# miguelmartin75/txt2vid

Measured on AMD Instinct MI355X. Metric: TGANv2 GAN train throughput (G+D steps x global batch), 16x64x64 videos/sec, higher is better.
Workload: dtype f32; 1 GPU; BASELINE configs[1]: unconditional TGANv2 16x64x64x1, per-GPU batch 32, fp32, RSGAN + GP 0.5, Adam 2e-4 (0.5,0.999), 1 D + 1 G step, subsample_input pyramid 8/16/32/64; global_batch=32, per_gpu_batch=32, parallelism=dp1

## Files before the change

include/t2v_hip.h:

```cpp
#ifndef T2V_HIP_H
#define T2V_HIP_H

#include <stdint.h>

#ifdef __cplusplus
extern "C" {
#endif

#define T2V_OK 0
#define T2V_EINVAL (-1)
#define T2V_ELAUNCH (-2)

#define T2V_MAX_TAPS 27

typedef struct {
    int32_t N, Cin, D, H, W, Cout;
    int32_t ntaps;
    int8_t dz[T2V_MAX_TAPS], dy[T2V_MAX_TAPS], dx[T2V_MAX_TAPS];
    int8_t pad_[3];
} t2v_conv_geom;

#define T2V_MAX_GROUPS 8
typedef struct {
    const float* x;
// ... 56 lines not shown
    int8_t pad_[5];
    int64_t tap_stride;
    int64_t split_stride;
} t2v_wgrad_src;
typedef struct {
    float* dw;
    float* dbias;
    int64_t CoCi;
    int32_t T, Cout, nsrc;
    int32_t accum, accum_bias;
    int32_t kind;
    int32_t block_begin, nblocks;
    int32_t tap_major;
    int32_t pad_;
    t2v_wgrad_src src[T2V_WGRAD_MAX_SRC];
} t2v_wgrad_dest;
int t2v_conv_wgrad_grouped_partial(const t2v_conv_group* groups, int ngroups, int Cin, int Cout, int kD, int kH, int kW,
                                   float* slab, int want_bias, int flags, t2v_wgrad_src* out_src, void* stream);
int t2v_wgrad_dest_bytes(void);
int t2v_wgrad_reduce_multi(const void* table , int ndest, int total_blocks, void* stream);

int t2v_conv_fwd_plan(const t2v_conv_group* groups, int ngroups, int Cin, int Cout, int flags, int32_t* out);
int t2v_conv_wgrad_plan(const t2v_conv_group* groups, int ngroups, int Cin, int Cout, int kD, int kH, int kW, int32_t* out);
int64_t t2v_conv_wgrad_grouped_bias_slab_floats(const t2v_conv_group* groups, int ngroups, int Cin, int Cout, int kD,
                                                int kH, int kW);
int t2v_conv_wgrad_grouped_bias(const t2v_conv_group* groups, int ngroups, int Cin, int Cout, int kD, int kH, int kW,
                                float* dw, float* dbias, float* slab, int flags, void* stream);

int t2v_pack_weight_bf16(const float* w, void* wpb, int Cout, int Cin, int T, const int32_t* taps, int ntaps, int mode, void* stream);
int t2v_conv_fwd_grouped_bf16_ok(const t2v_conv_group* groups, int ngroups, int Cin, int Cout);
int t2v_conv_fwd_bf16_plan(const t2v_conv_group* groups, int ngroups, int Cin, int Cout, int flags, int32_t* out);
int t2v_conv_fwd_grouped_bf16(const t2v_conv_group* groups, int ngroups, int Cin, int Cout, const void* wpb, const float* bias,
                              float* ws, int flags, void* stream);

int64_t t2v_channel_sum_ws_floats(int N, int C, int64_t S);
int t2v_channel_sum(const float* x, float* out, float* ws, int N, int C, int64_t S, int accum, void* stream);
int64_t t2v_channel_sum_grouped_ws_floats(const t2v_conv_group* groups, int ngroups, int C);
int t2v_channel_sum_grouped(const t2v_conv_group* groups, int ngroups, int C, float* out, float* ws, int accum, void* stream);

int t2v_relu(const float* x, float* y, int64_t n, void* stream);
int t2v_relu_mask(const float* g, const float* x, float* gx, int64_t n, void* stream);
int t2v_add(const float* a, const float* b, float* y, int64_t n, void* stream);
int t2v_axpby(float alpha, const float* a, float beta, const float* b, float* y, int64_t n, void* stream);
int t2v_scale_dev(const float* s, float mul, const float* a, float* y, int64_t n, void* stream);
int t2v_dot(const float* a, const float* b, float* out, float* ws , int64_t n, int accum, void* stream);
int t2v_fill(float* y, float v, int64_t n, void* stream);
// ... 225 lines not shown
```

txt2vid_amd/_lib.py:

```python
import ctypes as C
import os

_HERE = os.path.dirname(os.path.abspath(__file__))
LIB_PATH = os.environ.get('T2V_LIB') or os.path.join(_HERE, 'csrc', 'libt2v_hip.so')

MAX_TAPS = 27


class ConvGeom(C.Structure):
    _fields_ = [('N', C.c_int32), ('Cin', C.c_int32), ('D', C.c_int32), ('H', C.c_int32), ('W', C.c_int32),
                ('Cout', C.c_int32), ('ntaps', C.c_int32),
                ('dz', C.c_int8 * MAX_TAPS), ('dy', C.c_int8 * MAX_TAPS), ('dx', C.c_int8 * MAX_TAPS),
                ('pad_', C.c_int8 * 3)]


class ConvGroup(C.Structure):
    _fields_ = [('x', C.c_void_p), ('y', C.c_void_p), ('mask', C.c_void_p), ('N', C.c_int32), ('D', C.c_int32), ('H', C.c_int32), ('W', C.c_int32),
                ('ntaps', C.c_int32), ('dstride', C.c_int32), ('ydstride', C.c_int32), ('yoff', C.c_int32), ('Dy', C.c_int32),
                ('dz', C.c_int8 * MAX_TAPS), ('dy', C.c_int8 * MAX_TAPS), ('dx', C.c_int8 * MAX_TAPS), ('widx', C.c_int8 * MAX_TAPS)]


class AdamJob(C.Structure):
    _fields_ = [('p', C.c_void_p), ('g', C.c_void_p), ('m', C.c_void_p), ('v', C.c_void_p), ('n', C.c_int64)]

# ... 52 lines not shown
_F = C.c_float
_I3 = C.POINTER(C.c_int32)
_G = C.POINTER(ConvGeom)

SIGNATURES = {
    't2v_pack_weight': [_P, _P, _I, _I, _I, _I3, _I, _I, _P],
    't2v_pack_job_bytes': [],
    't2v_pack_multi': [_P, _I, _I, _P],
    't2v_pack_weight_into': [_P, _P, _I, _I, _I, _I3, _I, _I, _I, _I, _I, _I, _P],
    't2v_conv_fwd': [_P, _P, _P, _P, _P, _G, _I, _P],
    't2v_conv_fwd_ws_floats': [_G],
    't2v_conv_wgrad_slab_floats': [_G, _I],
    't2v_conv_fwd_grouped_ws_floats': [_P, _I, _I, _I],
    't2v_conv_fwd_grouped': [_P, _I, _I, _I, _P, _P, _P, _I, _P],
    't2v_conv_wgrad_grouped_slab_floats': [_P, _I, _I, _I, _I, _I, _I],
    't2v_conv_fwd_plan': [_P, _I, _I, _I, _I, _I3],
    't2v_nonlocal_ok': [_I, _I],
    't2v_nonlocal_fwd': [_P, _P, _P, _P, _P, _I, _I, _I, _I, _I, _P],
    't2v_nonlocal_bwd': [_P, _P, _P, _P, _P, _P, _P, _P, _P, _P, _I, _I, _I, _I, _I, _P],
    't2v_conv_wgrad_grouped_partial': [_P, _I, _I, _I, _I, _I, _I, _P, _I, _I, _P, _P],
    't2v_wgrad_dest_bytes': [],
    't2v_wgrad_reduce_multi': [_P, _I, _I, _P],
    't2v_conv_wgrad_plan': [_P, _I, _I, _I, _I, _I, _I, _I3],
    't2v_pack_weight_bf16': [_P, _P, _I, _I, _I, _P, _I, _I, _P],
    't2v_conv_fwd_grouped_bf16_ok': [_P, _I, _I, _I],
    't2v_conv_fwd_bf16_plan': [_P, _I, _I, _I, _I, _I3],
    't2v_conv_fwd_grouped_bf16': [_P, _I, _I, _I, _P, _P, _P, _I, _P],
    't2v_conv_wgrad_grouped': [_P, _I, _I, _I, _I, _I, _I, _P, _P, _I, _P],
    't2v_conv_wgrad_grouped_bias_slab_floats': [_P, _I, _I, _I, _I, _I, _I],
    't2v_conv_wgrad_grouped_bias': [_P, _I, _I, _I, _I, _I, _I, _P, _P, _P, _I, _P],
    't2v_conv_wgrad': [_P, _P, _P, _P, _G, _I3, _I, _I, _P],
    't2v_channel_sum_ws_floats': [_I, _I, _L],
    't2v_channel_sum': [_P, _P, _P, _I, _I, _L, _I, _P],
    't2v_channel_sum_grouped_ws_floats': [_P, _I, _I],
    't2v_channel_sum_grouped': [_P, _I, _I, _P, _P, _I, _P],
    't2v_relu': [_P, _P, _L, _P],
    't2v_relu_mask': [_P, _P, _P, _L, _P],
    't2v_add': [_P, _P, _P, _L, _P],
    't2v_axpby': [_F, _P, _F, _P, _P, _L, _P],
    't2v_scale_dev': [_P, _F, _P, _P, _L, _P],
    't2v_dot': [_P, _P, _P, _P, _L, _I, _P],
    't2v_fill': [_P, _F, _L, _P],
    't2v_tanh': [_P, _P, _L, _P],
    't2v_tanh_bwd': [_P, _P, _P, _L, _P],
    't2v_avgpool3d': [_P, _P, _P, _I, _I, _I, _I, _I, _I, _I, _I3, _I3, _I3, _P],
    't2v_avgpool3d_bwd': [_P, _P, _I, _I, _I, _I, _I, _I, _I, _I3, _I3, _I3, _P],
# ... 125 lines not shown
```

txt2vid_amd/csrc/conv.hip:

```cpp
#include <hip/hip_runtime.h>
#include <stdint.h>
#include "../../include/t2v_hip.h"

typedef float f32x16 __attribute__((ext_vector_type(16)));

#ifdef T2V_STAMPS
__device__ unsigned long long* g_stamps = nullptr;
__device__ unsigned int g_stamps_cap = 0;
extern "C" int t2v_stamps_set(void* buf, unsigned int cap_records) {
    if (hipMemcpyToSymbol(HIP_SYMBOL(g_stamps), &buf, sizeof(buf)) != hipSuccess) return -1;
    if (hipMemcpyToSymbol(HIP_SYMBOL(g_stamps_cap), &cap_records, sizeof(cap_records)) != hipSuccess) return -1;
    return 0;
}
__device__ __forceinline__ unsigned long long stamp_now() {
    unsigned long long t;
    __builtin_amdgcn_sched_barrier(0);
    asm volatile("s_memtime %0\n\ts_waitcnt lgkmcnt(0)" : "=s"(t) :: "memory");
    __builtin_amdgcn_sched_barrier(0);
    return t;
}
#define STAMP(v) const unsigned long long v = stamp_now()
#define STAMP_ACC(acc, a, b) acc += (b) - (a)
#else
#define STAMP(v)
// ... 3503 lines not shown
            const int slot = col / Cin, ci = col - slot * Cin;
            float* ps = slab + ((size_t)split * live.n + slot) * Cout * Cin + ci;
#pragma unroll
            for (int r = 0; r < 16; ++r) {
                const int co = co0 + wco * 32 + (r & 3) + 8 * (r >> 2) + 4 * hi;
                if (co < Cout) ps[(size_t)co * Cin] = acc[r];
            }
        } else if (col == 31 && bias_slab != nullptr) {
#pragma unroll
            for (int r = 0; r < 16; ++r) {
                const int co = co0 + wco * 32 + (r & 3) + 8 * (r >> 2) + 4 * hi;
                if (co < Cout) bias_slab[(size_t)split * Cout + co] = acc[r];
            }
        }
    }
}

#define W3_AP (WG_BK + 1)
#define W3_BP (WG_BK + 3)
struct LiveRows { int8_t r[9]; int32_t n; };

#define W3_XP (WG_BK + 3)

template <bool BF16>
__global__ __launch_bounds__(256, BF16 ? 4 : 0) void conv_wgrad3_kernel(const WGroupTable tab, float* __restrict__ slab, const int Cin,
                                                          const int Cout, const int kD, const int kH, const int flags,
                                                          const int chunks_per_split, const LiveRows live,
                                                          float* __restrict__ bias_slab) {
    constexpr int LDS_A = BF16 ? 64 * B16_KP * 2 : 64 * W3_AP * 4;
    constexpr int LDS_B = BF16 ? 3 * 64 * B16_KP * 2 : 3 * 64 * W3_XP * 4;
    __shared__ __attribute__((aligned(16))) unsigned char lds_raw[LDS_A + LDS_B];
    float* const As = reinterpret_cast<float*>(lds_raw);
    float* const Bs = reinterpret_cast<float*>(lds_raw + LDS_A);
    __bf16* const Ah = reinterpret_cast<__bf16*>(lds_raw);
    __bf16* const Bh = reinterpret_cast<__bf16*>(lds_raw + LDS_A);
    const int tid = threadIdx.x, lane = tid & 63, wave = tid >> 6;
    const int l31 = lane & 31, hi = lane >> 5;
    const int wco = wave & 1, wci = wave >> 1;
    const int nco_t = (Cout + 63) / 64;
    const int co0 = (blockIdx.x % nco_t) * 64, ci0 = (blockIdx.x / nco_t) * 64;
    const int lin = xcd_remap((int)(blockIdx.y + blockIdx.z * gridDim.y), (int)(gridDim.y * gridDim.z));
    const int rslot = lin % (int)gridDim.y;
    const int split = lin / (int)gridDim.y;
    const int krow = live.r[rslot];
    const int dz = krow / kH - kD / 2, dy = krow % kH - kH / 2;
    const float relu_floor = (flags & T2V_CONV_RELU_IN) ? 0.f : -__builtin_inff();
    const int ml = tid & 31, rl = tid >> 5;
    const bool full = co0 + 64 <= Cout && ci0 + 64 <= Cin;

    f32x16 acc0, acc1, acc2;
#pragma unroll
    for (int r = 0; r < 16; ++r) { acc0[r] = 0.f; acc1[r] = 0.f; acc2[r] = 0.f; }

// ... 78 lines not shown
                ra[p] = __builtin_bit_cast(float, __builtin_amdgcn_raw_buffer_load_b32(g_y, oa, p * sty, 0));
                rb[p] = __builtin_bit_cast(float, __builtin_amdgcn_raw_buffer_load_b32(g_x, ob, p * st, 0));
            }
        } else {
#pragma unroll
            for (int p = 0; p < 8; ++p) {
                const int co = co0 + rl + p * 8, ci = ci0 + rl + p * 8;
                ra[p] = __builtin_bit_cast(float, __builtin_amdgcn_raw_buffer_load_b32(
                    g_y, (gbase + (uint32_t)(co < Cout ? co : Cout - 1) * uDHWo) * 4u, 0, 0));
                rb[p] = __builtin_bit_cast(float, __builtin_amdgcn_raw_buffer_load_b32(
                    g_x, (xb + (uint32_t)(ci < Cin ? ci : Cin - 1) * uDHW) * 4u, 0, 0));
            }
        }
        const uint32_t xb_l = __shfl(xb, 0, 64), xb_r = __shfl(xb, 31, 64);
        if (tid < 128) {
            const int row = tid >> 1, side = tid & 1;
            const int ci = ci0 + row;
            const uint32_t base = side ? (((pm2 >> 31) & 1u) ? xb_r + 1u : 0u) : ((pm0 & 1u) ? xb_l - 1u : 0u);
            rh = __builtin_bit_cast(float, __builtin_amdgcn_raw_buffer_load_b32(
                g_x, (base + (uint32_t)(ci < Cin ? ci : Cin - 1) * uDHW) * 4u, 0, 0));
        }
    };

    if (q0 < q1) load_chunk(q0);
    for (int q = q0; q < q1; ++q) {
        {
            const bool v0 = (((uint64_t)pm0 >> (ml + 1)) & 1u) != 0;
            const bool v1 = ((pm1 >> ml) & 1u) != 0;
            const bool v2 = ((((uint64_t)pm2 << 1) >> ml) & 1u) != 0;
            if (do_bias) {
#pragma unroll
                for (int p = 0; p < 8; ++p) bsum[p] += pend_mv ? ra[p] : 0.f;
            }
            if constexpr (BF16) {
                const int c_m1 = ml + 1, c_p1 = ml >= 1 ? ml - 1 : 33;
#pragma unroll
                for (int p = 0; p < 8; ++p) {
                    const int row = rl + p * 8;
                    float a = ra[p], v = fmaxf(rb[p], relu_floor);
                    if (!full) {
                        a = (co0 + row < Cout) ? a : 0.f;
                        v = (ci0 + row < Cin) ? v : 0.f;
                    }
                    Ah[row * B16_KP + ml] = (__bf16)a;
                    Bh[(0 * 64 + row) * B16_KP + c_m1] = (__bf16)(v0 ? v : 0.f);
                    Bh[(1 * 64 + row) * B16_KP + ml] = (__bf16)(v1 ? v : 0.f);
// ... 49 lines not shown
#pragma unroll
        for (int k2 = 0; k2 < WG_BK / 2; ++k2) {
            const float a = qa[k2 * 2];
            const float b0 = qb[0 * 64 * W3_XP + k2 * 2];
            const float b1 = qb[1 * 64 * W3_XP + k2 * 2];
            const float b2 = qb[2 * 64 * W3_XP + k2 * 2];
            acc0 = __builtin_amdgcn_mfma_f32_32x32x2f32(a, b0, acc0, 0, 0, 0);
            acc1 = __builtin_amdgcn_mfma_f32_32x32x2f32(a, b1, acc1, 0, 0, 0);
            acc2 = __builtin_amdgcn_mfma_f32_32x32x2f32(a, b2, acc2, 0, 0, 0);
        }
        }
        __syncthreads();
    }
    if (do_bias) {
#pragma unroll
        for (int p = 0; p < 8; ++p) {
            float v = bsum[p];
#pragma unroll
            for (int o = 16; o > 0; o >>= 1) v += __shfl_xor(v, o, 64);
            const int co = co0 + rl + p * 8;
            if (ml == 0 && co < Cout) bias_slab[(size_t)split * Cout + co] = v;
        }
    }
    const int ci = ci0 + wci * 32 + l31;
    if (ci < Cin) {
        const size_t CoCi = (size_t)Cout * Cin;
        float* ps = slab + ((size_t)split * (live.n * 3) + (size_t)rslot * 3) * CoCi + ci;
#pragma unroll
        for (int r = 0; r < 16; ++r) {
            const int co = co0 + wco * 32 + (r & 3) + 8 * (r >> 2) + 4 * hi;
            if (co < Cout) {
                ps[(size_t)co * Cin] = acc0[r];
                ps[CoCi + (size_t)co * Cin] = acc1[r];
                ps[2 * CoCi + (size_t)co * Cin] = acc2[r];
            }
        }
    }
}


__global__ __launch_bounds__(256, 4) void conv_pool_wgrad_kernel(const WGroupTable tab, float* __restrict__ slab, const int Cin,
                                                              const int Cout, const int chunks_per_split, const LiveRows live,
                                                              float* __restrict__ bias_slab) {
    constexpr int PA = WG_BK + 1;
    __shared__ __attribute__((aligned(16))) float As[64 * PA];
    __shared__ __attribute__((aligned(16))) float Bs[3 * 64 * PA];
    const int tid = threadIdx.x, lane = tid & 63, wave = tid >> 6;
    const int l31 = lane & 31, hi = lane >> 5;
    const int wco = wave & 1, wci = wave >> 1;
    const int nco_t = (Cout + 63) / 64;
    const int co0 = (blockIdx.x % nco_t) * 64, ci0 = (blockIdx.x / nco_t) * 64;
    const int lin = xcd_remap((int)(blockIdx.y + blockIdx.z * gridDim.y), (int)(gridDim.y * gridDim.z));
    const int rslot = lin % (int)gridDim.y;
    const int split = lin / (int)gridDim.y;
    const int krow = live.r[rslot];
    const int dz = krow / 3 - 1, dy = krow % 3 - 1;
    const int ml = tid & 31, rl = tid >> 5;
    const bool full = co0 + 64 <= Cout && ci0 + 64 <= Cin;

    f32x16 acc0, acc1, acc2;
#pragma unroll
    for (int r = 0; r < 16; ++r) { acc0[r] = 0.f; acc1[r] = 0.f; acc2[r] = 0.f; }

    const int nchunks = tab.chunk_start[tab.n];
    const int q0 = split * chunks_per_split;
    int q1 = q0 + chunks_per_split;
    if (q1 > nchunks) q1 = nchunks;

    float ra[8], rb1[8];
// ... 62 lines not shown
        const uint32_t uVp = (uint32_t)gVp, uVn = (uint32_t)gVn;
        if (full) {
            const uint32_t oa = (gbase + (uint32_t)(co0 + rl) * uVn) * 4u, ob = (xb + (uint32_t)(ci0 + rl) * uVp) * 4u;
            const int st = 32 * gVp, sty = 32 * gVn;
#pragma unroll
            for (int p = 0; p < 8; ++p) {
                ra[p] = __builtin_bit_cast(float, __builtin_amdgcn_raw_buffer_load_b32(g_y, oa, p * sty, 0));
                rb2[p] = __builtin_bit_cast(float2, __builtin_amdgcn_raw_buffer_load_b64(g_x, ob, p * st, 0));
                rb1[p] = __builtin_bit_cast(float, __builtin_amdgcn_raw_buffer_load_b32(g_x, ob + 8u, p * st, 0));
            }
        } else {
#pragma unroll
            for (int p = 0; p < 8; ++p) {
                const int co = co0 + rl + p * 8, ci = ci0 + rl + p * 8;
                ra[p] = __builtin_bit_cast(float, __builtin_amdgcn_raw_buffer_load_b32(
                    g_y, (gbase + (uint32_t)(co < Cout ? co : Cout - 1) * uVn) * 4u, 0, 0));
                const uint32_t ob = (xb + (uint32_t)(ci < Cin ? ci : Cin - 1) * uVp) * 4u;
                rb2[p] = __builtin_bit_cast(float2, __builtin_amdgcn_raw_buffer_load_b64(g_x, ob, 0, 0));
                rb1[p] = __builtin_bit_cast(float, __builtin_amdgcn_raw_buffer_load_b32(g_x, ob + 8u, 0, 0));
            }
        }
    };

    if (q0 < q1) load_chunk(q0);
    for (int q = q0; q < q1; ++q) {
        {
            if (do_bias) {
#pragma unroll
                for (int p = 0; p < 8; ++p) bsum[p] += pend_mv ? ra[p] : 0.f;
            }
            float* pa = &As[rl * PA + ml];
            float* pb = &Bs[rl * PA + ml];
#pragma unroll
            for (int p = 0; p < 8; ++p) {
                float a = pend_mv ? ra[p] : 0.f;
                float v0 = pend_vc ? rb2[p].x : 0.f, v1 = pend_vc ? rb2[p].y : 0.f, v2 = pend_vc ? rb1[p] : 0.f;
                if (!full) {
                    const int row = rl + p * 8;
                    a = (co0 + row < Cout) ? a : 0.f;
                    const bool ok = ci0 + row < Cin;
                    v0 = ok ? v0 : 0.f; v1 = ok ? v1 : 0.f; v2 = ok ? v2 : 0.f;
                }
                pa[p * 8 * PA] = a;
                pb[(0 * 64 + p * 8) * PA] = v0;
                pb[(1 * 64 + p * 8) * PA] = v1;
                pb[(2 * 64 + p * 8) * PA] = v2;
// ... 4 lines not shown
        const float* qa = &As[(wco * 32 + l31) * PA + hi];
        const float* qb = &Bs[(wci * 32 + l31) * PA + hi];
#pragma unroll
        for (int k2 = 0; k2 < WG_BK / 2; ++k2) {
            const float a = qa[k2 * 2];
            const float b0 = qb[0 * 64 * PA + k2 * 2];
            const float b1 = qb[1 * 64 * PA + k2 * 2];
            const float b2 = qb[2 * 64 * PA + k2 * 2];
            acc0 = __builtin_amdgcn_mfma_f32_32x32x2f32(a, b0, acc0, 0, 0, 0);
            acc1 = __builtin_amdgcn_mfma_f32_32x32x2f32(a, b1, acc1, 0, 0, 0);
            acc2 = __builtin_amdgcn_mfma_f32_32x32x2f32(a, b2, acc2, 0, 0, 0);
        }
        __syncthreads();
    }
    if (do_bias) {
#pragma unroll
        for (int p = 0; p < 8; ++p) {
            float v = bsum[p];
#pragma unroll
            for (int o = 16; o > 0; o >>= 1) v += __shfl_xor(v, o, 64);
            const int co = co0 + rl + p * 8;
            if (ml == 0 && co < Cout) bias_slab[(size_t)split * Cout + co] = v;
        }
    }
    const int ci = ci0 + wci * 32 + l31;
    if (ci < Cin) {
        const size_t CoCi = (size_t)Cout * Cin;
        float* ps = slab + ((size_t)split * (live.n * 3) + (size_t)rslot * 3) * CoCi + ci;
#pragma unroll
        for (int r = 0; r < 16; ++r) {
            const int co = co0 + wco * 32 + (r & 3) + 8 * (r >> 2) + 4 * hi;
            if (co < Cout) {
                ps[(size_t)co * Cin] = acc0[r];
                ps[CoCi + (size_t)co * Cin] = acc1[r];
                ps[2 * CoCi + (size_t)co * Cin] = acc2[r];
            }
        }
    }
}


__device__ __forceinline__ void bias_slab_reduce(const float* __restrict__ bias_slab, float* __restrict__ dbias, int S, int Cout,
                                                 int accum) {
    for (int co = threadIdx.x; co < Cout; co += 256) {
        float v0 = 0.f, v1 = 0.f, v2 = 0.f, v3 = 0.f;
        int s = 0;
// ... 167 lines not shown
    for (int i = 0; i < 2; ++i)
#pragma unroll
        for (int j = 0; j < 2; ++j) {
            const int ci = ci0 + wci * 64 + j * 32 + l31;
#pragma unroll
            for (int r = 0; r < 16; ++r) {
                const int co = co0 + wco * 64 + i * 32 + (r & 3) + 8 * (r >> 2) + 4 * hi;
                if (co < Cout && ci < Cin) out[(size_t)co * Cin + ci] = acc[i][j][r];
            }
        }
    if (do_bias) {
        float* red = As;
        *reinterpret_cast<float4*>(&red[r8 * WGM_AP + c4]) = bsum;
        __syncthreads();
        if (tid < 128 && co0 + tid < Cout) {
            float v = 0.f;
#pragma unroll
            for (int k = 0; k < 8; ++k) v += red[k * WGM_AP + tid];
            bias_slab[(size_t)split * Cout + co0 + tid] = v;
        }
    }
}

struct WgradPlan { int S, cps; uint32_t live; int nlive; long nchunks; bool rows3; uint32_t liverows; int nrows; bool strided; bool gemm; bool thin; };

static bool build_wtable(const t2v_conv_group* groups, int ngroups, int Cin, int Cout, int kD, int kH, int kW, bool need_ptrs,
                         WGroupTable& tab, WgradPlan& p) {
    if (!groups || ngroups < 1 || ngroups > T2V_MAX_GROUPS || Cin < 1 || Cout < 1) return false;
    if ((kD != 1 && kD != 3) || (kH != 1 && kH != 3) || (kW != 1 && kW != 3)) return false;
    long nch = 0, maxMC = 0;
    bool strided = false;
    p.live = 0;
    tab.n = ngroups;
    for (int i = 0; i < ngroups; ++i) {
        const t2v_conv_group& g = groups[i];
        if (need_ptrs && (!g.x || !g.y)) return false;
        if (g.N < 1 || g.D < 1 || g.H < 1 || g.W < 1 || g.dstride < 0 || g.dstride > 2 || g.ydstride > 1 || g.ydstride < 0) return false;
        if (g.dstride == 2) strided = true;
        const long M = (long)g.N * g.D * g.H * g.W;
        if (M * (long)(Cin > Cout ? Cin : Cout) >= (1L << 30)) return false;
        if (M * (long)(Cin > Cout ? Cin : Cout) > maxMC) maxMC = M * (long)(Cin > Cout ? Cin : Cout);
        tab.g[i] = g;
        tab.chunk_start[i] = (int32_t)nch;
        nch += ((long)g.N * out_frames(g) * g.H * g.W + WG_BK - 1) / WG_BK;
        for (int a = 0; a < kD; ++a) for (int b = 0; b < kH; ++b) for (int c = 0; c < kW; ++c) {
            const int dz = a - kD / 2, dy = b - kH / 2, dx = c - kW / 2;
// ... 69 lines not shown
}

static void fill_wgrad_plan(int Cin, int Cout, const WgradPlan& p, int32_t* out) {
    const long tiles = (long)((Cout + 63) / 64) * ((Cin + 63) / 64);
    out[0] = p.gemm ? 3 : p.rows3 ? 2 : p.thin ? 4 : (Cin < 64 ? 1 : 0);
    out[1] = p.S;
    out[2] = p.cps;
    out[3] = p.nlive;
    out[4] = ((long)Cout * Cin <= 16384 && p.S >= 16) ? 1 : 0;
    if (p.gemm) { out[5] = (int32_t)((long)((Cout + 127) / 128) * ((Cin + 127) / 128) * p.S); return; }
    if (p.thin) { out[5] = (int32_t)((long)((Cout + 63) / 64) * p.S); return; }
    out[5] = (int32_t)((p.rows3 ? tiles * p.nrows : Cin < 64 ? (long)((Cout + 63) / 64) * (((long)p.nlive * Cin + 63) / 64)
                                                              : tiles * p.nlive) * p.S);
}
extern "C" int t2v_conv_wgrad_plan(const t2v_conv_group* groups, int ngroups, int Cin, int Cout, int kD, int kH, int kW,
                                   int32_t* out) {
    WGroupTable tab;
    WgradPlan p;
    if (!out || !build_wtable(groups, ngroups, Cin, Cout, kD, kH, kW, false, tab, p)) return T2V_EINVAL;
    fill_wgrad_plan(Cin, Cout, p, out);
    return T2V_OK;
}

extern "C" int64_t t2v_channel_sum_grouped_ws_floats(const t2v_conv_group* groups, int ngroups, int C);
extern "C" int t2v_channel_sum_grouped(const t2v_conv_group* groups, int ngroups, int C, float* out, float* ws, int accum, void* stream);

static int64_t wgrad_bias_extra(const t2v_conv_group* groups, int ngroups, int Cin, int Cout, const WgradPlan& p) {
    return (int64_t)p.S * Cout;
}
extern "C" int64_t t2v_conv_wgrad_grouped_bias_slab_floats(const t2v_conv_group* groups, int ngroups, int Cin, int Cout, int kD,
                                                           int kH, int kW) {
    WGroupTable tab;
    WgradPlan p;
    if (!build_wtable(groups, ngroups, Cin, Cout, kD, kH, kW, false, tab, p)) return T2V_EINVAL;
    return (int64_t)p.S * p.nlive * Cout * Cin + wgrad_bias_extra(groups, ngroups, Cin, Cout, p);
}

static int wgrad_impl(const t2v_conv_group* groups, int ngroups, int Cin, int Cout, int kD, int kH, int kW, float* dw,
                      float* dbias, float* slab, int flags, void* stream, t2v_wgrad_src* out_src = nullptr);
extern "C" int t2v_conv_wgrad_grouped(const t2v_conv_group* groups, int ngroups, int Cin, int Cout, int kD, int kH, int kW,
                                      float* dw, float* slab, int flags, void* stream) {
    return wgrad_impl(groups, ngroups, Cin, Cout, kD, kH, kW, dw, nullptr, slab, flags, stream);
}
extern "C" int t2v_conv_wgrad_grouped_bias(const t2v_conv_group* groups, int ngroups, int Cin, int Cout, int kD, int kH, int kW,
                                           float* dw, float* dbias, float* slab, int flags, void* stream) {
    if (!dbias) return T2V_EINVAL;
// ... 36 lines not shown
    for (int i = 0; i < ngroups; ++i) {
        int live_g = 0;
        for (int a = 0; a < kD; ++a) for (int b = 0; b < kH; ++b) for (int c = 0; c < kW; ++c) {
            const int dz = a - kD / 2, dy = b - kH / 2, dx = c - kW / 2;
            if (!((groups[i].D == 1 && dz) || (groups[i].H == 1 && dy) || (groups[i].W == 1 && dx))) ++live_g;
        }
        flops += 2.0 * (double)groups[i].N * out_frames(groups[i]) * groups[i].H * groups[i].W * Cout * Cin * live_g;
    }
    {
        ProfScope prof(1, flops, s, p.nchunks * WG_BK, Cin, Cout, live.n, ngroups, p.S);
        int32_t plan_[8] = {-1, -1, -1, -1, -1, -1, -1, -1};
        fill_wgrad_plan(Cin, Cout, p, plan_);
        plan_[6] = ((flags & T2V_CONV_BF16) && !p.gemm && (p.rows3 || Cin >= 64)) ? 1 : 0;
        plan_[7] = p.strided ? 1 : 0;
        ProfScope::set_plan(plan_, 8);
        if (p.gemm) {
            dim3 grid((unsigned)(((Cout + 127) / 128) * ((Cin + 127) / 128)), 1u, (unsigned)p.S);
            T2V_LAUNCH_PROF(conv_wgrad_gemm_kernel, grid, dim3(256), 0, s, tab, slab, Cin, Cout, flags, p.cps,
                            dbias ? bias_part : (float*)nullptr);
        } else if (p.rows3) {
            dim3 grid((unsigned)(((Cout + 63) / 64) * ((Cin + 63) / 64)), (unsigned)lrows.n, (unsigned)p.S);
            if (flags & T2V_CONV_BF16)
                T2V_LAUNCH_PROF(conv_wgrad3_kernel<true>, grid, dim3(256), 0, s, tab, slab, Cin, Cout, kD, kH, flags, p.cps, lrows,
                                dbias ? bias_part : (float*)nullptr);
            else
                T2V_LAUNCH_PROF(conv_wgrad3_kernel<false>, grid, dim3(256), 0, s, tab, slab, Cin, Cout, kD, kH, flags, p.cps, lrows,
                                dbias ? bias_part : (float*)nullptr);
        } else if (Cin < 64 && p.thin) {
            dim3 grid((unsigned)((Cout + 63) / 64), 1u, (unsigned)p.S);
            T2V_LAUNCH_PROF(conv_wgrad_thin_kernel, grid, dim3(256), 0, s, tab, slab, Cin, Cout, T, kH, kW, flags, p.cps, live,
                            dbias ? bias_part : (float*)nullptr);
        } else if (Cin < 64) {
            dim3 grid((unsigned)(((Cout + 63) / 64) * ((live.n * Cin + 63) / 64)), 1u, (unsigned)p.S);
            T2V_LAUNCH_PROF(conv_wgrad_cols_kernel, grid, dim3(256), 0, s, tab, slab, Cin, Cout, T, kH, kW, flags, p.cps, live,
                            dbias ? bias_part : (float*)nullptr);
        } else {
            dim3 grid((unsigned)(((Cout + 63) / 64) * ((Cin + 63) / 64)), (unsigned)live.n, (unsigned)p.S);
            if (flags & T2V_CONV_BF16)
                T2V_LAUNCH_PROF(conv_wgrad_bf16_kernel, grid, dim3(256), 0, s, tab, slab, Cin, Cout, T, kH, kW, flags, p.cps, live,
                                dbias ? bias_part : (float*)nullptr);
            else
                T2V_LAUNCH_PROF(conv_wgrad_kernel, grid, dim3(256), 0, s, tab, slab, Cin, Cout, T, kH, kW, flags, p.cps, live,
                                dbias ? bias_part : (float*)nullptr);
        }
    }
    int st = launch_status();
// ... 242 lines not shown
    if ((!dw && !out_src) || !slab || !build_pool_wtable(groups, ngroups, Cin, Cout, kD, true, tab, p)) return T2V_EINVAL;
    hipStream_t s = (hipStream_t)stream;
    float* bias_part = slab + (size_t)p.S * p.nlive * Cout * Cin;
    const int T = kD * 9;
    TapMap map;
    for (int t = 0; t < T2V_MAX_TAPS; ++t) map.j[t] = -1;
    LiveRows lrows;
    lrows.n = 0;
    for (int r = 0; r < 9; ++r) lrows.r[r] = 0;
    for (int r = 0; r < 9; ++r)
        if ((p.liverows >> r) & 1u) {
            const int rw = kD == 3 ? r : r - 3;
            for (int c = 0; c < 3; ++c) map.j[rw * 3 + c] = lrows.n * 3 + c;
            lrows.r[lrows.n++] = (int8_t)r;
        }
    double flops = 0;
    for (int i = 0; i < ngroups; ++i) flops += 2.0 * (double)pool_rows(groups[i]) * Cout * Cin * (groups[i].dstride ? 27 : 9);
    {
        ProfScope prof(1, flops, s, p.nchunks * WG_BK, Cin, Cout, p.nlive, ngroups, p.S);
        int32_t plan_[8] = {11, p.S, p.cps, p.nlive, ((long)Cout * Cin <= 16384 && p.S >= 16) ? 1 : 0,
                            (int32_t)((long)((Cout + 63) / 64) * ((Cin + 63) / 64) * p.nrows * p.S), 0, 0};
        ProfScope::set_plan(plan_, 8);
        dim3 grid((unsigned)(((Cout + 63) / 64) * ((Cin + 63) / 64)), (unsigned)lrows.n, (unsigned)p.S);
        T2V_LAUNCH_PROF(conv_pool_wgrad_kernel, grid, dim3(256), 0, s, tab, slab, Cin, Cout, p.cps, lrows, want_bias ? bias_part : (float*)nullptr);
    }
    int st = launch_status();
    if (st) return st;
    if (out_src) {
        out_src->slab = slab;
        out_src->bias_slab = want_bias ? bias_part : (const float*)nullptr;
        out_src->ntaps = p.nlive;
        out_src->S = p.S;
        out_src->tap_stride = (int64_t)Cout * Cin;
        out_src->split_stride = (int64_t)p.nlive * Cout * Cin;
        for (int t = 0; t < T2V_MAX_TAPS; ++t) out_src->map[t] = (int8_t)(t < T ? map.j[t] : -1);
        return T2V_OK;
    }
    const float* bias_in = want_bias ? bias_part : (const float*)nullptr;
    const int accum_bias = (flags & T2V_CONV_ACCUM_BIAS) ? 1 : 0;
    const long CoCi = (long)Cout * Cin;
    ProfScope prof2(2, 0.0, s, CoCi, Cin, Cout, T, p.nlive, p.S);
    if (CoCi <= 16384 && p.S >= 16)
        T2V_LAUNCH_PROF(wgrad_reduce_small_kernel, dim3((unsigned)((CoCi + 63) / 64), (unsigned)T), dim3(256), 0, s, slab, dw, CoCi, T,
                   p.nlive, p.S, map, (flags & T2V_CONV_ACCUM) ? 1 : 0, bias_in, dbias, Cout, accum_bias);
    else
        T2V_LAUNCH_PROF(wgrad_reduce_kernel, dim3((unsigned)((CoCi + 63) / 64)), dim3(256), 0, s, slab, dw, CoCi, T, p.nlive, p.S, map,
                   (flags & T2V_CONV_ACCUM) ? 1 : 0, bias_in, dbias, Cout, accum_bias);
// ... 7 lines not shown
extern "C" int t2v_pool_conv_wgrad_partial(const t2v_conv_group* groups, int ngroups, int Cin, int Cout, int kD, float* slab,
                                           int want_bias, int flags, t2v_wgrad_src* out_src, void* stream) {
    if (!out_src) return T2V_EINVAL;
    return pool_wgrad_impl(groups, ngroups, Cin, Cout, kD, nullptr, nullptr, want_bias != 0, slab, flags, stream, out_src);
}
extern "C" int t2v_pool_conv_plan(int what, const t2v_conv_group* groups, int ngroups, int Cin, int Cout, int32_t* out) {
    if (!out) return T2V_EINVAL;
    for (int i = 0; i < 8; ++i) out[i] = 0;
    if (what == 0 || what == 1) {
        GroupTable tab;
        PoolPlan p;
        if (!(what == 0 ? build_pool_fwd(groups, ngroups, Cin, Cout, false, tab, p) : build_pool_dgrad(groups, ngroups, Cin, Cout, false, tab, p)))
            return T2V_EINVAL;
        const bool db = what == 0 ? pool_fwd_db() : pool_dgrad_db();
        out[0] = what == 0 ? 9 : 10; out[1] = 64; out[2] = 64; out[3] = db ? 16 : 32; out[4] = 1; out[5] = p.vecb ? 1 : 0; out[6] = db ? 2 : 1; out[7] = p.S;
        return T2V_OK;
    }
    if (what == 2) {
        WGroupTable tab;
        WgradPlan p;
        if (!build_pool_wtable(groups, ngroups, Cin, Cout, 3, false, tab, p)) return T2V_EINVAL;
        out[0] = 11; out[1] = p.S; out[2] = p.cps; out[3] = p.nlive; out[4] = ((long)Cout * Cin <= 16384 && p.S >= 16) ? 1 : 0;
        out[5] = (int32_t)((long)((Cout + 63) / 64) * ((Cin + 63) / 64) * p.nrows * p.S);
        return T2V_OK;
    }
    return T2V_EINVAL;
}

extern "C" int t2v_wgrad_dest_bytes(void) { return (int)sizeof(t2v_wgrad_dest); }


__global__ __launch_bounds__(256) void wgrad_reduce_multi_kernel(const t2v_wgrad_dest* __restrict__ table, int ndest) {
    __shared__ __attribute__((aligned(16))) float tile[256 * T2V_MAX_TAPS];
    __shared__ __attribute__((aligned(16))) float part[4][256];
    __shared__ int s_dest;
    if (threadIdx.x == 0) {
        int lo = 0, hi = ndest - 1;
        while (lo < hi) {
            const int mid = (lo + hi + 1) >> 1;
            if (table[mid].block_begin <= (int)blockIdx.x) lo = mid; else hi = mid - 1;
        }
        s_dest = lo;
    }
    __syncthreads();
    const t2v_wgrad_dest& d = table[s_dest];
    const int b = (int)blockIdx.x - d.block_begin;
// ... 304 lines not shown
```

Before: 3004 videos/s.

## Double-buffer fp32 wgrad and pool-wgrad kernels with half-chunk software pipelining

Adds a double-buffered variant of the fp32 3-row wgrad kernel and the pooled wgrad kernel. Each K chunk is split into two half-chunk rounds with two LDS buffers, so global loads for the next round are issued between MFMAs and staged into the other buffer. This needs only one barrier per round, where the single-buffer version waits on a load then stage then compute sequence. It is on by default through T2V_WGRAD_DB and adds launch bounds of 4, which may raise register pressure. A plan query reporting the chosen form is also exposed.

After: 3000 videos/s. No clear change (-0.1%).

```diff
diff --git a/include/t2v_hip.h b/include/t2v_hip.h
--- a/include/t2v_hip.h
+++ b/include/t2v_hip.h
@@ -102,6 +102,7 @@
 
 int t2v_conv_fwd_plan(const t2v_conv_group* groups, int ngroups, int Cin, int Cout, int flags, int32_t* out);
 int t2v_conv_wgrad_plan(const t2v_conv_group* groups, int ngroups, int Cin, int Cout, int kD, int kH, int kW, int32_t* out);
+int t2v_conv_wgrad_round_form(const t2v_conv_group* groups, int ngroups, int Cin, int Cout, int kD, int kH, int kW, int flags);
 int64_t t2v_conv_wgrad_grouped_bias_slab_floats(const t2v_conv_group* groups, int ngroups, int Cin, int Cout, int kD,
                                                 int kH, int kW);
 int t2v_conv_wgrad_grouped_bias(const t2v_conv_group* groups, int ngroups, int Cin, int Cout, int kD, int kH, int kW,
diff --git a/txt2vid_amd/_lib.py b/txt2vid_amd/_lib.py
--- a/txt2vid_amd/_lib.py
+++ b/txt2vid_amd/_lib.py
@@ -98,6 +98,7 @@
     't2v_wgrad_dest_bytes': [],
     't2v_wgrad_reduce_multi': [_P, _I, _I, _P],
     't2v_conv_wgrad_plan': [_P, _I, _I, _I, _I, _I, _I, _I3],
+    't2v_conv_wgrad_round_form': [_P, _I, _I, _I, _I, _I, _I, _I],
     't2v_pack_weight_bf16': [_P, _P, _I, _I, _I, _P, _I, _I, _P],
     't2v_conv_fwd_grouped_bf16_ok': [_P, _I, _I, _I],
     't2v_conv_fwd_bf16_plan': [_P, _I, _I, _I, _I, _I3],
diff --git a/txt2vid_amd/csrc/conv.hip b/txt2vid_amd/csrc/conv.hip
--- a/txt2vid_amd/csrc/conv.hip
+++ b/txt2vid_amd/csrc/conv.hip
@@ -3549,13 +3549,14 @@
 
 #define W3_XP (WG_BK + 3)
 
-template <bool BF16>
-__global__ __launch_bounds__(256, BF16 ? 4 : 0) void conv_wgrad3_kernel(const WGroupTable tab, float* __restrict__ slab, const int Cin,
+template <bool BF16, bool DB = false>
+__global__ __launch_bounds__(256, (BF16 || DB) ? 4 : 0) void conv_wgrad3_kernel(const WGroupTable tab, float* __restrict__ slab, const int Cin,
                                                           const int Cout, const int kD, const int kH, const int flags,
                                                           const int chunks_per_split, const LiveRows live,
                                                           float* __restrict__ bias_slab) {
-    constexpr int LDS_A = BF16 ? 64 * B16_KP * 2 : 64 * W3_AP * 4;
-    constexpr int LDS_B = BF16 ? 3 * 64 * B16_KP * 2 : 3 * 64 * W3_XP * 4;
+    static_assert(!(BF16 && DB), "the double-buffered round is fp32 only");
+    constexpr int LDS_A = BF16 ? 64 * B16_KP * 2 : DB ? 2 * 64 * (WG_BK / 2 + 1) * 4 : 64 * W3_AP * 4;
+    constexpr int LDS_B = BF16 ? 3 * 64 * B16_KP * 2 : DB ? 2 * 3 * 64 * (WG_BK / 2 + 3) * 4 : 3 * 64 * W3_XP * 4;
     __shared__ __attribute__((aligned(16))) unsigned char lds_raw[LDS_A + LDS_B];
     float* const As = reinterpret_cast<float*>(lds_raw);
     float* const Bs = reinterpret_cast<float*>(lds_raw + LDS_A);
@@ -3680,6 +3681,160 @@
         }
     };
 
+    if constexpr (DB) {
+        constexpr int HK = WG_BK / 2;
+        constexpr int AP2 = HK + 1, XP2 = HK + 3;
+        constexpr int ASZ = 64 * AP2, BSZ = 3 * 64 * XP2;
+        float* const A2 = As;
+        float* const B2 = As + 2 * ASZ;
+        const int hl = tid & (HK - 1), hr = tid >> 4;
+        const bool halo_thread = tid < 128;
+        const int hrow = halo_thread ? (tid >> 1) : (tid & 63), hside = tid & 1;
+        const int hci = ci0 + hrow < Cin ? ci0 + hrow : Cin - 1;
+        const bool hrow_ok = halo_thread && ci0 + hrow < Cin;
+        const int halo_dst = halo_thread ? (hside ? (2 * 64 + hrow) * XP2 + HK : hrow * XP2 + 1) : hrow * XP2 + HK + 2;
+        const int r0 = 2 * q0, r1 = 2 * q1;
+        float ra2[2][4], rb2[2][4], rh2[2] = {0.f, 0.f};
+        uint32_t m0s[2] = {0u, 0u}, m1s[2] = {0u, 0u}, m2s[2] = {0u, 0u};
+        bool mvb[2] = {false, false};
+        float bsum2[2][4];
+#pragma unroll
+        for (int p = 0; p < 4; ++p) { bsum2[0][p] = 0.f; bsum2[1][p] = 0.f; ra2[0][p] = ra2[1][p] = rb2[0][p] = rb2[1][p] = 0.f; }
+        uint32_t l_oa = 0u, l_ob = 0u, l_oh = 0u, l_gb = 0u, l_xb = 0u, l_DHW = 1u, l_DHWo = 1u;
+        auto prep = [&](int st, int r) {
+            const int rr = r < r1 ? r : r1 - 1;
+            const int q = rr >> 1;
+            if (q >= g_end || g_i < 0) enter_group(q);
+            const int D = gD, H = gH, W = gW, HW = gHW, DHW = gDHW, DHWo = gDHWo;
+            const int m = (q - g_begin) * WG_BK + (rr & 1) * HK + hl;
+            const bool mv = m < gM;
+            int n, spo, d_o, h, w_;
+            if (g_pow2) {
+                n = m >> g_lo;
+                spo = m & (DHWo - 1);
+                d_o = spo >> g_lhw;
+                h = (spo >> g_lw) & (H - 1);
+                w_ = spo & (W - 1);
+            } else {
+                const bool small = gM < (1 << 24);
+                n = small ? fast_div(m, DHWo, 1.0f / (float)DHWo) : m / DHWo;
+                spo = m - n * DHWo;
+                d_o = small ? fast_div(spo, HW, 1.0f / (float)HW) : spo / HW;
+                const int rem = spo - d_o * HW;
+                h = small ? fast_div(rem, W, 1.0f / (float)W) : rem / W;
+                w_ = rem - h * W;
+            }
+            const int d = d_o * g_ds;
+            const int sp = spo + d_o * (g_ds - 1) * HW;
+            const bool vc = mv && (unsigned)(d + dz) < (unsigned)D && (unsigned)(h + dy) < (unsigned)H;
+            const uint32_t gbase = mv ? (uint32_t)(n * DHWo) * (uint32_t)Cout + (uint32_t)spo : 0u;
+            const uint32_t xb = vc ? (uint32_t)(n * DHW) * (uint32_t)Cin + (uint32_t)(sp + g_shift) : 0u;
+            const uint32_t p0 = (uint32_t)__ballot(vc && w_ >= 1) & 0xffffu, p1 = (uint32_t)__ballot(vc) & 0xffffu,
+                           p2 = (uint32_t)__ballot(vc && w_ + 1 < W) & 0xffffu;
+            m0s[st] = p0; m1s[st] = p1; m2s[st] = p2;
+            mvb[st] = mv && do_bias && r < r1;
+            l_DHW = (uint32_t)DHW; l_DHWo = (uint32_t)DHWo;
+            l_gb = gbase; l_xb = xb;
+            l_oa = (gbase + (uint32_t)(co0 + hr) * l_DHWo) * 4u;
+            l_ob = (xb + (uint32_t)(ci0 + hr) * l_DHW) * 4u;
+            const uint32_t xb_l = __shfl(xb, 0, 64), xb_r = __shfl(xb, HK - 1, 64);
+            const uint32_t hb = hside ? (((p2 >> (HK - 1)) & 1u) ? xb_r + 1u : 0u) : ((p0 & 1u) ? xb_l - 1u : 0u);
+            l_oh = halo_thread ? (hb + (uint32_t)hci * l_DHW) * 4u : 0u;
+        };
+        auto load_item = [&](auto FULL, int st, int i) {
+            constexpr bool fullc = decltype(FULL)::value;
+            if (i < 8) {
+                const int p = i >> 1;
+                if (fullc) {
+                    if (i & 1) rb2[st][p] = __builtin_bit_cast(float, __builtin_amdgcn_raw_buffer_load_b32(g_x, l_ob, p * 64 * (int)l_DHW, 0));
+                    else ra2[st][p] = __builtin_bit_cast(float, __builtin_amdgcn_raw_buffer_load_b32(g_y, l_oa, p * 64 * (int)l_DHWo, 0));
+                } else {
+                    const int co = co0 + hr + p * 16, ci = ci0 + hr + p * 16;
+                    if (i & 1) rb2[st][p] = __builtin_bit_cast(float, __builtin_amdgcn_raw_buffer_load_b32(
+                                   g_x, (l_xb + (uint32_t)(ci < Cin ? ci : Cin - 1) * l_DHW) * 4u, 0, 0));
+                    else ra2[st][p] = __builtin_bit_cast(float, __builtin_amdgcn_raw_buffer_load_b32(
+                                   g_y, (l_gb + (uint32_t)(co < Cout ? co : Cout - 1) * l_DHWo) * 4u, 0, 0));
+                }
+            } else if (i == 8) rh2[st] = __builtin_bit_cast(float, __builtin_amdgcn_raw_buffer_load_b32(g_x, l_oh, 0, 0));
+        };
+        auto stage_item = [&](auto FULL, int st, float* A, float* B, int p) {
+            constexpr bool fullc = decltype(FULL)::value;
+            if (p < 4) {
+                const bool v0 = ((m0s[st] >> (hl + 1)) & 1u) != 0;
+                const bool v1 = ((m1s[st] >> hl) & 1u) != 0;
+                const bool v2 = (((m2s[st] << 1) >> hl) & 1u) != 0;
+                bsum2[st][p] += mvb[st] ? ra2[st][p] : 0.f;
+                float a = ra2[st][p], v = fmaxf(rb2[st][p], relu_floor);
+                if (!fullc) {
+                    const int row = hr + p * 16;
+                    a = (co0 + row < Cout) ? a : 0.f;
+                    v = (ci0 + row < Cin) ? v : 0.f;
+                }
+                A[(hr + p * 16) * AP2 + hl] = a;
+                float* pb = &B[(hr + p * 16) * XP2 + 1 + hl];
+                pb[0 * 64 * XP2 + 1] = v0 ? v : 0.f;
+                pb[1 * 64 * XP2] = v1 ? v : 0.f;
+                pb[2 * 64 * XP2 - 1] = v2 ? v : 0.f;
+            } else {
+                const bool ok = hrow_ok && (hside ? ((m2s[st] >> (HK - 1)) & 1u) != 0 : (m0s[st] & 1u) != 0);
+                B[halo_dst] = ok ? fmaxf(rh2[st], relu_floor) : 0.f;
+            }
+        };
+        auto round = [&](auto FULL, auto CUR, int r) {
+            constexpr int cur = decltype(CUR)::value, nxt = cur ^ 1;
+            prep(cur, r + 2);
+            const float* qa = A2 + cur * ASZ + (wco * 32 + l31) * AP2 + hi;
+            const float* qb = B2 + cur * BSZ + (wci * 32 + l31) * XP2 + 1 + hi;
+            float* An = A2 + nxt * ASZ;
+            float* Bn = B2 + nxt * BSZ;
+#pragma unroll
+            for (int k2 = 0; k2 < HK / 2; ++k2) {
+                const float a = qa[k2 * 2];
+                const float b0 = qb[0 * 64 * XP2 + k2 * 2];
+                const float b1 = qb[1 * 64 * XP2 + k2 * 2];
+                const float b2 = qb[2 * 64 * XP2 + k2 * 2];
+                acc0 = __builtin_amdgcn_mfma_f32_32x32x2f32(a, b0, acc0, 0, 0, 0);
+                if (k2 < 3) load_item(FULL, cur, k2 * 3 + 0);
+                acc1 = __builtin_amdgcn_mfma_f32_32x32x2f32(a, b1, acc1, 0, 0, 0);
+                if (k2 < 3) load_item(FULL, cur, k2 * 3 + 1);
+                acc2 = __builtin_amdgcn_mfma_f32_32x32x2f32(a, b2, acc2, 0, 0, 0);
+                if (k2 < 3) load_item(FULL, cur, k2 * 3 + 2);
+                if (k2 >= 3 && k2 < 7) stage_item(FULL, nxt, An, Bn, k2 - 3);
+                if (k2 == 7) stage_item(FULL, nxt, An, Bn, 4);
+                if (k2 == 2 || k2 == 6) __builtin_amdgcn_sched_barrier(0);
+            }
+            __syncthreads();
+        };
+        auto run = [&](auto FULL) {
+            if (r0 < r1) {
+                prep(0, r0);
+#pragma unroll
+                for (int i = 0; i < 9; ++i) load_item(FULL, 0, i);
+                prep(1, r0 + 1);
+#pragma unroll
+                for (int i = 0; i < 9; ++i) load_item(FULL, 1, i);
+#pragma unroll
+                for (int p = 0; p < 5; ++p) stage_item(FULL, 0, A2, B2, p);
+            }
+            __syncthreads();
+            for (int r = r0; r < r1; r += 2) {
+                round(FULL, std::integral_constant<int, 0>{}, r);
+                round(FULL, std::integral_constant<int, 1>{}, r + 1);
+            }
+        };
+        if (full) run(std::true_type{});
+        else run(std::false_type{});
+        if (do_bias) {
+#pragma unroll
+            for (int p = 0; p < 4; ++p) {
+                float v = bsum2[0][p] + bsum2[1][p];
+#pragma unroll
+                for (int o = 8; o > 0; o >>= 1) v += __shfl_xor(v, o, 64);
+                const int co = co0 + hr + p * 16;
+                if (hl == 0 && co < Cout) bias_slab[(size_t)split * Cout + co] = v;
+            }
+        }
+    } else {
     if (q0 < q1) load_chunk(q0);
     for (int q = q0; q < q1; ++q) {
         {
@@ -3775,6 +3930,7 @@
             if (ml == 0 && co < Cout) bias_slab[(size_t)split * Cout + co] = v;
         }
     }
+    }
     const int ci = ci0 + wci * 32 + l31;
     if (ci < Cin) {
         const size_t CoCi = (size_t)Cout * Cin;
@@ -3792,12 +3948,13 @@
 }
 
 
+template <bool DB>
 __global__ __launch_bounds__(256, 4) void conv_pool_wgrad_kernel(const WGroupTable tab, float* __restrict__ slab, const int Cin,
                                                               const int Cout, const int chunks_per_split, const LiveRows live,
                                                               float* __restrict__ bias_slab) {
-    constexpr int PA = WG_BK + 1;
-    __shared__ __attribute__((aligned(16))) float As[64 * PA];
-    __shared__ __attribute__((aligned(16))) float Bs[3 * 64 * PA];
+    constexpr int PA = DB ? WG_BK / 2 + 1 : WG_BK + 1;
+    __shared__ __attribute__((aligned(16))) float As[(DB ? 2 : 1) * 64 * PA];
+    __shared__ __attribute__((aligned(16))) float Bs[(DB ? 2 : 1) * 3 * 64 * PA];
     const int tid = threadIdx.x, lane = tid & 63, wave = tid >> 6;
     const int l31 = lane & 31, hi = lane >> 5;
     const int wco = wave & 1, wci = wave >> 1;
@@ -3906,6 +4063,139 @@
         }
     };
 
+    if constexpr (DB) {
+        constexpr int HK = WG_BK / 2;
+        constexpr int ASZ = 64 * PA, BSZ = 3 * 64 * PA;
+        const int hl = tid & (HK - 1), hr = tid >> 4;
+        const int r0 = 2 * q0, r1 = 2 * q1;
+        float ra2[2][4], rc2[2][4];
+        float2 rd2[2][4];
+        bool mv2[2] = {false, false}, vc2[2] = {false, false}, mvb[2] = {false, false};
+        float bsum2[2][4];
+#pragma unroll
+        for (int p = 0; p < 4; ++p) {
+            bsum2[0][p] = bsum2[1][p] = ra2[0][p] = ra2[1][p] = rc2[0][p] = rc2[1][p] = 0.f;
+            rd2[0][p] = rd2[1][p] = make_float2(0.f, 0.f);
+        }
+        uint32_t l_oa = 0u, l_ob = 0u, l_gb = 0u, l_xb = 0u, l_Vp = 1u, l_Vn = 1u;
+        auto prep = [&](int st, int r) {
+            const int rr = r < r1 ? r : r1 - 1;
+            const int q = rr >> 1;
+            if (q >= g_end || g_i < 0) enter_group(q);
+            const int m = (q - g_begin) * WG_BK + (rr & 1) * HK + hl;
+            const bool mv = m < gM;
+            int n, sp, e, i, j;
+            if (g_pow2) {
+                n = m >> g_lv;
+                sp = m & (gVn - 1);
+                e = sp >> g_lhw;
+                i = (sp >> g_lw) & (gHn - 1);
+                j = sp & (gWn - 1);
+            } else {
+                const bool small = gM < (1 << 24);
+                n = small ? fast_div(m, gVn, 1.0f / (float)gVn) : m / gVn;
+                sp = m - n * gVn;
+                e = small ? fast_div(sp, gHWn, 1.0f / (float)gHWn) : sp / gHWn;
+                const int rem = sp - e * gHWn;
+                i = small ? fast_div(rem, gWn, 1.0f / (float)gWn) : rem / gWn;
+                j = rem - i * gWn;
+            }
+            const bool vc = mv && (g_tm != 0 || dz == 0);
+            l_gb = mv ? (uint32_t)(n * gVn) * (uint32_t)Cout + (uint32_t)sp : 0u;
+            l_xb = vc ? (uint32_t)(n * gVp) * (uint32_t)Cin +
+                            (uint32_t)(((g_tm ? 2 * e + dz + 1 : 0) * gHp + 2 * i + dy + 1) * gWp + 2 * j) : 0u;
+            mv2[st] = mv; vc2[st] = vc;
+            mvb[st] = mv && do_bias && r < r1;
+            l_Vp = (uint32_t)gVp; l_Vn = (uint32_t)gVn;
+            l_oa = (l_gb + (uint32_t)(co0 + hr) * l_Vn) * 4u;
+            l_ob = (l_xb + (uint32_t)(ci0 + hr) * l_Vp) * 4u;
+        };
+        auto load_item = [&](auto FULL, int st, int i) {
+            constexpr bool fullc = decltype(FULL)::value;
+            const int p = i / 3, w = i - p * 3;
+            uint32_t oa = l_oa, ob = l_ob;
+            int so_a = p * 64 * (int)l_Vn, so_b = p * 64 * (int)l_Vp;
+            if (!fullc) {
+                const int co = co0 + hr + p * 16, ci = ci0 + hr + p * 16;
+                oa = (l_gb + (uint32_t)(co < Cout ? co : Cout - 1) * l_Vn) * 4u;
+                ob = (l_xb + (uint32_t)(ci < Cin ? ci : Cin - 1) * l_Vp) * 4u;
+                so_a = so_b = 0;
+            }
+            if (w == 0) ra2[st][p] = __builtin_bit_cast(float, __builtin_amdgcn_raw_buffer_load_b32(g_y, oa, so_a, 0));
+            else if (w == 1) rd2[st][p] = __builtin_bit_cast(float2, __builtin_amdgcn_raw_buffer_load_b64(g_x, ob, so_b, 0));
+            else rc2[st][p] = __builtin_bit_cast(float, __builtin_amdgcn_raw_buffer_load_b32(g_x, ob + 8u, so_b, 0));
+        };
+        auto stage_item = [&](auto FULL, int st, float* A, float* B, int p) {
+            constexpr bool fullc = decltype(FULL)::value;
+            bsum2[st][p] += mvb[st] ? ra2[st][p] : 0.f;
+            float a = mv2[st] ? ra2[st][p] : 0.f;
+            float v0 = vc2[st] ? rd2[st][p].x : 0.f, v1 = vc2[st] ? rd2[st][p].y : 0.f, v2 = vc2[st] ? rc2[st][p] : 0.f;
+            if (!fullc) {
+                const int row = hr + p * 16;
+                a = (co0 + row < Cout) ? a : 0.f;
+                const bool ok = ci0 + row < Cin;
+                v0 = ok ? v0 : 0.f; v1 = ok ? v1 : 0.f; v2 = ok ? v2 : 0.f;
+            }
+            A[(hr + p * 16) * PA + hl] = a;
+            float* pb = &B[(hr + p * 16) * PA + hl];
+            pb[0 * 64 * PA] = v0;
+            pb[1 * 64 * PA] = v1;
+            pb[2 * 64 * PA] = v2;
+        };
+        auto round = [&](auto FULL, auto CUR, int r) {
+            constexpr int cur = decltype(CUR)::value, nxt = cur ^ 1;
+            prep(cur, r + 2);
+            const float* qa = As + cur * ASZ + (wco * 32 + l31) * PA + hi;
+            const float* qb = Bs + cur * BSZ + (wci * 32 + l31) * PA + hi;
+            float* An = As + nxt * ASZ;
+            float* Bn = Bs + nxt * BSZ;
+#pragma unroll
+            for (int k2 = 0; k2 < HK / 2; ++k2) {
+                const float a = qa[k2 * 2];
+                const float b0 = qb[0 * 64 * PA + k2 * 2];
+                const float b1 = qb[1 * 64 * PA + k2 * 2];
+                const float b2 = qb[2 * 64 * PA + k2 * 2];
+                acc0 = __builtin_amdgcn_mfma_f32_32x32x2f32(a, b0, acc0, 0, 0, 0);
+                if (k2 < 4) load_item(FULL, cur, k2 * 3 + 0);
+                acc1 = __builtin_amdgcn_mfma_f32_32x32x2f32(a, b1, acc1, 0, 0, 0);
+                if (k2 < 4) load_item(FULL, cur, k2 * 3 + 1);
+                acc2 = __builtin_amdgcn_mfma_f32_32x32x2f32(a, b2, acc2, 0, 0, 0);
+                if (k2 < 4) load_item(FULL, cur, k2 * 3 + 2);
+                if (k2 >= 4) stage_item(FULL, nxt, An, Bn, k2 - 4);
+                if (k2 == 3 || k2 == 7) __builtin_amdgcn_sched_barrier(0);
+            }
+            __syncthreads();
+        };
+        auto run = [&](auto FULL) {
+            if (r0 < r1) {
+                prep(0, r0);
+#pragma unroll
+                for (int i = 0; i < 12; ++i) load_item(FULL, 0, i);
+                prep(1, r0 + 1);
+#pragma unroll
+                for (int i = 0; i < 12; ++i) load_item(FULL, 1, i);
+#pragma unroll
+                for (int p = 0; p < 4; ++p) stage_item(FULL, 0, As, Bs, p);
+            }
+            __syncthreads();
+            for (int r = r0; r < r1; r += 2) {
+                round(FULL, std::integral_constant<int, 0>{}, r);
+                round(FULL, std::integral_constant<int, 1>{}, r + 1);
+            }
+        };
+        if (full) run(std::true_type{});
+        else run(std::false_type{});
+        if (do_bias) {
+#pragma unroll
+            for (int p = 0; p < 4; ++p) {
+                float v = bsum2[0][p] + bsum2[1][p];
+#pragma unroll
+                for (int o = 8; o > 0; o >>= 1) v += __shfl_xor(v, o, 64);
+                const int co = co0 + hr + p * 16;
+                if (hl == 0 && co < Cout) bias_slab[(size_t)split * Cout + co] = v;
+            }
+        }
+    } else {
     if (q0 < q1) load_chunk(q0);
     for (int q = q0; q < q1; ++q) {
         {
@@ -3956,6 +4246,7 @@
             const int co = co0 + rl + p * 8;
             if (ml == 0 && co < Cout) bias_slab[(size_t)split * Cout + co] = v;
         }
+    }
     }
     const int ci = ci0 + wci * 32 + l31;
     if (ci < Cin) {
@@ -4169,6 +4460,7 @@
     }
 }
 
+static bool wgrad_db() { static const bool v = env_long("T2V_WGRAD_DB", 1) != 0; return v; }
 struct WgradPlan { int S, cps; uint32_t live; int nlive; long nchunks; bool rows3; uint32_t liverows; int nrows; bool strided; bool gemm; bool thin; };
 
 static bool build_wtable(const t2v_conv_group* groups, int ngroups, int Cin, int Cout, int kD, int kH, int kW, bool need_ptrs,
@@ -4284,6 +4576,15 @@
     return T2V_OK;
 }
 
+extern "C" int t2v_conv_wgrad_round_form(const t2v_conv_group* groups, int ngroups, int Cin, int Cout, int kD, int kH, int kW,
+                                         int flags) {
+    WGroupTable tab;
+    WgradPlan p;
+    if (!build_wtable(groups, ngroups, Cin, Cout, kD, kH, kW, false, tab, p)) return T2V_EINVAL;
+    if (p.gemm || !p.rows3) return 0;
+    return ((flags & T2V_CONV_BF16) || !wgrad_db()) ? 1 : 2;
+}
+
 extern "C" int64_t t2v_channel_sum_grouped_ws_floats(const t2v_conv_group* groups, int ngroups, int C);
 extern "C" int t2v_channel_sum_grouped(const t2v_conv_group* groups, int ngroups, int C, float* out, float* ws, int accum, void* stream);
 
@@ -4366,6 +4667,9 @@
             dim3 grid((unsigned)(((Cout + 63) / 64) * ((Cin + 63) / 64)), (unsigned)lrows.n, (unsigned)p.S);
             if (flags & T2V_CONV_BF16)
                 T2V_LAUNCH_PROF(conv_wgrad3_kernel<true>, grid, dim3(256), 0, s, tab, slab, Cin, Cout, kD, kH, flags, p.cps, lrows,
+                                dbias ? bias_part : (float*)nullptr);
+            else if (wgrad_db())
+                T2V_LAUNCH_PROF((conv_wgrad3_kernel<false, true>), grid, dim3(256), 0, s, tab, slab, Cin, Cout, kD, kH, flags, p.cps, lrows,
                                 dbias ? bias_part : (float*)nullptr);
             else
                 T2V_LAUNCH_PROF(conv_wgrad3_kernel<false>, grid, dim3(256), 0, s, tab, slab, Cin, Cout, kD, kH, flags, p.cps, lrows,
@@ -4654,7 +4958,10 @@
                             (int32_t)((long)((Cout + 63) / 64) * ((Cin + 63) / 64) * p.nrows * p.S), 0, 0};
         ProfScope::set_plan(plan_, 8);
         dim3 grid((unsigned)(((Cout + 63) / 64) * ((Cin + 63) / 64)), (unsigned)lrows.n, (unsigned)p.S);
-        T2V_LAUNCH_PROF(conv_pool_wgrad_kernel, grid, dim3(256), 0, s, tab, slab, Cin, Cout, p.cps, lrows, want_bias ? bias_part : (float*)nullptr);
+        if (wgrad_db())
+            T2V_LAUNCH_PROF(conv_pool_wgrad_kernel<true>, grid, dim3(256), 0, s, tab, slab, Cin, Cout, p.cps, lrows, want_bias ? bias_part : (float*)nullptr);
+        else
+            T2V_LAUNCH_PROF(conv_pool_wgrad_kernel<false>, grid, dim3(256), 0, s, tab, slab, Cin, Cout, p.cps, lrows, want_bias ? bias_part : (float*)nullptr);
     }
     int st = launch_status();
     if (st) return st;
@@ -4708,6 +5015,7 @@
         if (!build_pool_wtable(groups, ngroups, Cin, Cout, 3, false, tab, p)) return T2V_EINVAL;
         out[0] = 11; out[1] = p.S; out[2] = p.cps; out[3] = p.nlive; out[4] = ((long)Cout * Cin <= 16384 && p.S >= 16) ? 1 : 0;
         out[5] = (int32_t)((long)((Cout + 63) / 64) * ((Cin + 63) / 64) * p.nrows * p.S);
+        out[6] = wgrad_db() ? 2 : 1;
         return T2V_OK;
     }
     return T2V_EINVAL;
```
